# microsoft/Cream

Hardware: AMD Instinct MI355X
Metric: images/sec (whole node) AutoFormer-S supernet step @224^2 (higher is better)
Workload: dtype bf16; 1 GPU; AutoFormer-S supernet train step, random-path sampling (random.seed(epoch)), per-GPU batch 128, 224x224, AdamW, grad all-reduce RCCL; global_batch=128, parallelism=dp1, wgrad_partials=bf16 split-K partial tiles (within 1.9e-3 of fp32 partials), mixup=on-device, in the timed region

## Files before the change

cream_amd/_lib.py:

```python
import ctypes
import os

_HERE = os.path.dirname(os.path.abspath(__file__))
LIB_PATH = os.path.join(_HERE, "libcream_amd.so")

CREAM_OK = 0
_ERRORS = {
    -1: "CREAM_ERR_BAD_ARG (null pointer, negative size or unsupported stride)",
    -2: "CREAM_ERR_BAD_DTYPE (element type not supported by this entry point)",
    -3: "CREAM_ERR_LAUNCH (HIP kernel launch failed)",
    -4: "CREAM_ERR_TOO_LARGE (shape exceeds what the kernel family supports)",
    -5: "CREAM_ERR_CHANNEL_STRIDE (the channel stride of a (B, H, W, C) view is not 1)",
    -6: "CREAM_ERR_BAD_STRIDE (a stride is negative, not a multiple of 8, or tokens overlap)",
    -7: "CREAM_ERR_BAD_SHAPE (a channel count or a map size outside the covered range)",
}

F32, F16, BF16, F64 = 0, 1, 2, 3


class CreamLibraryError(RuntimeError):
    pass


_c = ctypes
# ... 50 lines not shown
    "cream_token_dwconv3_bwd": (_i, [_vp, _vp]),
    "cream_token_dwconv7_part_size": (_i, [_i]),
    "cream_token_dwconv7_blocks": (_i, [_vp]),
    "cream_token_dwconv7_fwd": (_i, [_vp, _vp]),
    "cream_token_dwconv7_bwd": (_i, [_vp, _vp]),
    "cream_cga_attn_check": (_i, [_vp]),
    "cream_cga_attn_fwd": (_i, [_vp, _vp]),
    "cream_evit_dwffn_check": (_i, [_vp]),
    "cream_evit_dwffn_fwd": (_i, [_vp, _vp]),
    "cream_evit_pw_residual_check": (_i, [_vp]),
    "cream_evit_pw_residual_fwd": (_i, [_vp, _vp]),
    "cream_relation_loss_check": (_i, [_vp]),
    "cream_relation_loss_blocks": (_i, [_vp]),
    "cream_relation_loss": (_i, [_vp, _vp]),
    "cream_hidden_relation_check": (_i, [_vp]),
    "cream_hidden_relation_padded": (_i, [_i]),
    "cream_hidden_relation_parts": (_i, [_i, _i]),
    "cream_hidden_relation_loss": (_i, [_vp, _vp]),
    "cream_attn_rpe2d_padded_len": (_i, [_i]),
    "cream_attn_rpe2d_dtab_parts": (_i, [_i, _i]),
    "cream_attn_rpe2d_bwd_mode": (_i, [_i]),
    "cream_attn_rpe2d_fwd": (_i, [_vp, _vp, _vp, _vp, _vp, _vp, _i64, _i64, _i64, _vp, _vp, _vp, _vp, _i,
                                  _i, _i, _i, _i, _i, _i, _f, _i, _vp]),
    "cream_attn_rpe2d_bwd": (_i, [_vp, _vp, _vp, _i64, _i64, _i64, _vp, _vp, _vp, _vp, _vp,
                                  _vp, _vp, _vp, _vp, _vp, _vp, _vp, _i64, _i64, _i64,
                                  _vp, _vp, _vp, _vp, _i, _i, _i, _i, _i, _i, _i, _f, _i, _vp]),
    "cream_attn_rpe2d_fwd_img": (_i, [_vp, _vp, _vp, _vp, _vp, _vp, _i64, _i64, _i64, _vp, _vp, _vp, _vp, _i, _vp,
                                      _i, _i, _i, _i, _i, _i, _f, _i, _vp]),
    "cream_attn_rpe2d_bwd_img": (_i, [_vp, _vp, _vp, _i64, _i64, _i64, _vp, _vp, _vp, _vp, _vp,
                                      _vp, _vp, _vp, _vp, _vp, _vp, _vp, _i64, _i64, _i64,
                                      _vp, _vp, _vp, _vp, _i, _vp, _i, _i, _i, _i, _i, _i, _f, _i, _vp]),
    "cream_attn_rpe2d_fwd_drop": (_i, [_vp, _vp, _vp, _vp, _vp, _vp, _i64, _i64, _i64, _vp, _vp, _vp, _vp, _i, _vp,
                                       _i, _i, _i, _i, _i, _i, _f, _f, _c.c_uint32, _i, _vp]),
    "cream_attn_rpe2d_bwd_drop": (_i, [_vp, _vp, _vp, _i64, _i64, _i64, _vp, _vp, _vp, _vp, _vp,
                                       _vp, _vp, _vp, _vp, _vp, _vp, _vp, _i64, _i64, _i64,
                                       _vp, _vp, _vp, _vp, _i, _vp, _i, _i, _i, _i, _i, _i, _f, _f, _c.c_uint32, _i, _vp]),
    "cream_attn_rpe2d_table_image_bytes": (_i64, []),
    "cream_attn_rpe2d_table_images": (_i, [_vp, _vp, _vp, _vp, _vp, _i, _i, _vp]),
    "cream_attn_rpe2d_fwd_mode": (_i, [_i]),
    "cream_ln_fwd": (_i, [_vp, _vp, _vp, _vp, _vp, _vp, _i, _i, _f, _vp]),
    "cream_ln_partials": (_i, []),
    "cream_ln_bwd": (_i, [_vp, _vp, _vp, _vp, _vp, _vp, _vp, _vp, _vp, _vp, _i, _i, _i, _vp]),
    "cream_gelu_fwd": (_i, [_vp, _vp, _i64, _vp]),
    "cream_gelu_bwd": (_i, [_vp, _vp, _vp, _i64, _vp]),
    "cream_residual_add": (_i, [_vp, _vp, _vp, _vp, _i64, _i64, _vp]),
    "cream_scale_cast": (_i, [_vp, _vp, _vp, _i64, _i64, _vp]),
    "cream_colsum_slabs": (_i, [_i]),
    "cream_colsum": (_i, [_vp, _vp, _i, _i, _vp]),
    "cream_add_ln_fwd": (_i, [_vp, _vp, _vp, _vp, _vp, _vp, _vp, _i, _vp, _vp, _i, _i, _f, _vp]),
    "cream_block_wgrad_bf16": (_i, [_i]),
    "cream_colsum128_slabs": (_i, [_i]),
    "cream_colsum128": (_i, [_vp, _vp, _i, _i, _vp]),
    "cream_gelu_bwd_colsum": (_i, [_vp, _vp, _vp, _vp, _i, _i, _vp]),
    "cream_scale_cast_colsum": (_i, [_vp, _vp, _vp, _vp, _i, _i, _i, _vp]),
    "cream_grad_finalize": (_i, [_vp, _i, _vp]),
    "cream_ln_fwd_masked": (_i, [_vp, _vp, _vp, _vp, _vp, _vp, _vp, _i, _i, _i, _f, _vp]),
    "cream_add_ln_fwd_masked": (_i, [_vp, _vp, _vp, _vp, _vp, _vp, _vp, _i, _vp, _vp, _vp, _i, _i, _i, _f, _vp]),
    "cream_ln_bwd_masked": (_i, [_vp, _vp, _vp, _vp, _vp, _vp, _vp, _vp, _vp, _i, _vp, _vp, _i, _i, _i, _vp]),
    "cream_mask_pack_check": (_i, [_vp, _i]),
    "cream_mask_pack": (_i, [_vp, _i, _vp]),
    "cream_mask_grad_ws_floats": (_i64, [_i, _i]),
    "cream_mask_grad_check": (_i, [_vp, _i]),
    "cream_mask_grad_finalize": (_i, [_vp, _i, _vp]),
    "cream_grad_finalize_compact_check": (_i, [_vp, _i]),
    "cream_grad_finalize_compact": (_i, [_vp, _i, _vp]),
    "cream_pad_cols": (_i, [_vp, _vp, _i, _i, _i, _i, _vp]),
    "cream_unpad_cols": (_i, [_vp, _i, _vp, _i, _i, _i, _vp]),
    "cream_gemm_rows_per_colsum_slab": (_i, []),
    "cream_gemm_nt256": (_i, [_i]),
    "cream_gemm_nt8": (_i, [_i]),
    "cream_linear_fwd": (_i, [_vp, _vp, _vp, _vp, _i, _i, _i, _i64, _vp]),
    "cream_linear_fwd_seg": (_i, [_vp, _vp, _vp, _vp, _i, _i, _i, _i64, _i, _i64, _vp]),
    "cream_linear_gelu_fwd": (_i, [_vp, _vp, _vp, _vp, _vp, _i, _i, _i, _i64, _vp]),
    "cream_linear_gelu_fwd_pad": (_i, [_vp, _vp, _vp, _vp, _vp, _i, _i, _i, _i, _i64, _vp]),
    "cream_linear_dgrad": (_i, [_vp, _vp, _vp, _i, _i, _i, _i64, _vp]),
    "cream_linear_dgrad_seg": (_i, [_vp, _vp, _vp, _i, _i, _i, _i64, _i, _i64, _vp]),
    "cream_linear_dgrad_mul": (_i, [_vp, _vp, _vp, _vp, _vp, _i, _i, _i, _i64, _vp]),
    "cream_linear_wgrad_splits": (_i, [_i, _i, _i]),
    "cream_linear_wgrad_splits_bf16": (_i, [_i, _i, _i]),
    "cream_gemm_tn8": (_i, [_i]),
    "cream_gemm_nthalf": (_i, [_i]),
    "cream_gemm_nt224": (_i, [_i]),
    "cream_gemm_nt224_launches": (_i64, []),
    "cream_linear_nt224": (_i, [_vp, _vp, _vp, _vp, _i, _i, _i, _i64, _i, _i64, _i, _i64, _vp]),
    "cream_gemm_ntopt": (_i, [_i]),
    "cream_gemm_stagger": (_i, [_i]),
    "cream_block_layout_epoch": (_i, []),
    "cream_cu_reserve": (_i, [_i]),
    "cream_mixup_cutmix": (_i, [_vp, _vp, _vp, _i, _i, _i, _i, _i, _f, _i, _i, _i, _i, _i, _f, _vp]),
    "cream_image_batch_plan": (_i64, [_vp, _i, _i, _i]),
    "cream_image_batch_transform": (_i, [_vp, _vp, _i64, _vp, _vp, _i, _i, _i, _vp, _vp, _vp, _i64, _vp]),
    "cream_cu_count": (_i, []),
    "cream_linear_wgrad_parts": (_i, [_vp, _vp, _vp, _vp, _i, _i, _i, _i, _vp]),
    "cream_linear_wgrad_parts_bf16": (_i, [_vp, _vp, _vp, _vp, _i, _i, _i, _i, _vp]),
    "cream_param_job_tiles": (_i, [_i, _i]),
    "cream_adamw_step": (_i, [_vp, _vp, _i, _i, _i, _c.c_double, _c.c_double, _c.c_double, _c.c_double, _i64, _vp]),
    "cream_grad_clip_coef": (_i, [_vp, _vp, _i, _i, _c.c_double, _vp, _vp, _vp]),
    "cream_adamw_step_clipped": (_i, [_vp, _vp, _i, _i, _i, _c.c_double, _c.c_double, _c.c_double, _c.c_double, _i64, _vp, _vp]),
    "cream_grad_scale": (_i, [_vp, _vp, _i, _i, _vp, _vp]),
    "cream_adamw_step_groups": (_i, [_vp, _vp, _i, _i, _i, _vp, _vp, _i, _c.c_double, _c.c_double, _c.c_double, _i64, _vp, _vp]),
    "cream_soft_ce": (_i, [_vp, _vp, _vp, _vp, _i, _i, _i, _f, _vp]),
    "cream_sparse_ce": (_i, [_vp, _vp, _vp, _vp, _vp, _i, _i, _i, _i, _f, _vp]),
    "cream_softmax_topk_records": (_i, [_vp, _vp, _vp, _i, _i, _i, _i, _vp]),
    "cream_linear_f32_fwd": (_i, [_vp, _vp, _vp, _vp, _i, _i, _i, _i64, _i64, _i, _i, _vp]),
    "cream_bmm_f32": (_i, [_vp, _vp, _vp, _i, _i, _i, _vp, _vp, _vp, _i, _i, _vp]),
    "cream_linear_f32_dgrad": (_i, [_vp, _vp, _vp, _i, _i, _i, _i64, _i, _i, _vp]),
    "cream_linear_f32_wgrad": (_i, [_vp, _vp, _vp, _vp, _i, _i, _i, _i64, _i64, _i, _i, _vp]),
    "cream_ln_f32_fwd": (_i, [_vp, _vp, _vp, _vp, _vp, _vp, _i, _i, _f, _vp]),
    "cream_ln_f32_bwd": (_i, [_vp, _vp, _vp, _vp, _vp, _vp, _vp, _i, _i, _vp]),
    "cream_block_prof_enable": (_i, [_i]),
    "cream_block_prof_kinds": (_i, []),
    "cream_block_prof_name": (_c.c_char_p, [_i]),
    "cream_block_prof_collect": (_i, [_vp, _vp, _vp, _vp]),
    "cream_slices_copy": (_i, [_vp, _i, _vp, _i, _i, _vp]),
    "cream_block_fwd_workspace": (_i64, [_vp, _vp, _vp, _vp]),
    "cream_block_fwd": (_i, [_vp, _vp, _vp, _vp, _vp, _vp, _vp]),
    "cream_block_bwd_workspace": (_i64, [_vp, _vp, _vp, _vp]),
    "cream_block_bwd": (_i, [_vp, _vp, _vp, _vp, _vp, _vp, _vp, _vp, _i, _i64, _vp, _vp, _i, _vp, _vp]),
    "cream_image_augment_workspace": (_i64, [_i, _i, _i, _i]),
    "cream_image_augment_u8": (_i, [_vp, _vp, _i, _i, _i, _vp, _vp, _i, _vp, _i64, _vp]),
    "cream_image_batch_plan_aug": (_i64, [_vp, _i, _i, _i, _vp, _i]),
    "cream_image_batch_transform_aug": (_i, [_vp, _vp, _i64, _vp, _vp, _i, _i, _i, _vp, _vp, _vp, _vp, _i, _vp, _i64, _vp]),
}

MAX_GRAD_JOBS = 24
ADAMW_MAX_GROUPS = 64


class GradJob(ctypes.Structure):
    _fields_ = [("dst", _vp), ("src", _vp), ("ld", _i64), ("pstride", _i64),
                ("nparts", _c.c_int32), ("rows", _c.c_int32), ("cols", _c.c_int32),
                ("interleave", _c.c_int32), ("src_bf16", _c.c_int32), ("overwrite", _c.c_int32)]

MAX_MASK_JOBS = 16


class MaskPackJob(ctypes.Structure):
    _fields_ = ([(n, _vp) for n in ("w", "r", "c", "mir", "mir_t")] + [(n, _i64) for n in ("ld", "ld_mir", "ld_mir_t")] +
                [(n, _c.c_int32) for n in ("rows", "cols", "c_group", "reserved")])


class MaskGradJob(ctypes.Structure):
    _fields_ = ([(n, _vp) for n in ("dst", "src", "w", "r", "c", "dr_out", "dc_out", "ws")] +
                [(n, _i64) for n in ("ld", "pstride", "ld_w")] +
                [(n, _c.c_int32) for n in ("nparts", "rows", "cols", "c_group", "src_bf16", "overwrite", "dr_accumulate",
                                           "dc_accumulate")])


MAX_COMPACT_JOBS = 24


class GradCompactJob(ctypes.Structure):
    _fields_ = ([("dst", _vp), ("src", _vp)] + [(n, _i64) for n in ("ld_dst", "ld_src", "pstride")] +
                [(n, _c.c_int32) for n in ("nparts", "rows", "cols", "src_bf16", "overwrite", "reserved")])


class ImageDesc(ctypes.Structure):
    _fields_ = ([("offset", _i64)] +
                [(n, _c.c_int32) for n in ("height", "width", "row_stride", "box_top", "box_left", "box_h", "box_w", "resized_h",
                                           "resized_w", "win_top", "win_left", "flip", "row0", "nrows")] +
                [("tmp_off", _i64)] +
                [(n, _c.c_int32) for n in ("erase_top", "erase_left", "erase_h", "erase_w")] +
                [("erase_seed", _c.c_uint32), ("reserved", _c.c_int32)])


class AugOp(ctypes.Structure):
# ... 181 lines not shown
```

cream_amd/csrc/gemm_mfma.hip:

```cpp
#include <hip/hip_runtime.h>
#include <stdint.h>
#include <stdlib.h>
#include <atomic>

#include "cream_amd.h"
#include "gemm_mfma.hpp"
#include "gemm_nt8.hpp"
#include "gemm_nt224.hpp"
#include "gemm_tn8.hpp"
#include "launch_ev.hpp"
#include "cu_budget.hpp"
#include "env_switch.hpp"

namespace {
std::atomic<int> g_cu_reserve{0};
std::atomic<int> g_layout_epoch{0};
int physical_cus()
{
    static int cus = 0;
    if (!cus) {
        int dev = 0;
        hipDeviceProp_t prop;
        if (hipGetDevice(&dev) == hipSuccess && hipGetDeviceProperties(&prop, dev) == hipSuccess) cus = prop.multiProcessorCount;
        if (cus <= 0) cus = 256;
    }
    return cus;
}
}
namespace cream {
int cu_count()
{
    int c = (physical_cus() - g_cu_reserve.load(std::memory_order_relaxed)) / 8 * 8;
    return c < 8 ? 8 : c;
}
}

namespace {
using namespace cream;
using namespace cream::gemm;

int num_cus() { return cream::cu_count(); }

EnvSwitch g_nt256{"CREAM_GEMM_NT256", 2};
int nt256_mode() { return g_nt256.get(); }

EnvSwitch g_ntopt{"CREAM_GEMM_NTOPT", 3, [](int m) { return m & 15; }};
int ntopt_mode() { return g_ntopt.get(); }
EnvSwitch g_stagger{"CREAM_GEMM_STAGGER", 0};
int stagger_mode() { return g_stagger.get(); }

template <int EPI>
int launch_nt256(const NtParams& p, hipStream_t st)
{
    constexpr int BM = 256, BN = 256;
    auto kern = (ntopt_mode() & 4) ? gemm_nt_kernel<BM, BN, 2, 4, 2, EPI, 1, 1> : gemm_nt_kernel<BM, BN, 2, 4, 2, EPI, 1>;
    constexpr int lds = nt_lds_bytes(BM, BN, 2);
    if (!cream::raise_dynamic_lds(kern, lds)) return CREAM_ERR_LAUNCH;
    const int tiles = ((p.M + BM - 1) / BM) * ((p.N + BN - 1) / BN), slots = num_cus() / 8 * 8;
    CREAM_LAUNCH(kern, dim3(tiles < slots ? tiles : slots), dim3(512), lds, st, p);
    return hipGetLastError() == hipSuccess ? CREAM_OK : CREAM_ERR_LAUNCH;
}

EnvSwitch g_nt8{"CREAM_GEMM_NT8", 4};
int nt8_mode() { return g_nt8.get(); }

bool nt8_fits(const NtParams& p)
{
    const int64_t amax = (int64_t)p.M * p.lda, bmax = (int64_t)2 * p.nseg_stride + (int64_t)p.nseg * p.ldb + p.ldb;
    const int64_t bplain = (int64_t)p.N * p.ldb;
    return amax < ((int64_t)1 << 31) && bmax < ((int64_t)1 << 31) && bplain < ((int64_t)1 << 31) && p.lda < (1 << 24) && p.ldb < (1 << 24);
}

template <int EPI>
int launch_nt8(const NtParams& p, hipStream_t st)
{
    auto kern = gemm_nt8_kernel<EPI>;
    if (!cream::raise_dynamic_lds(kern, NT8_LDS_BYTES)) return CREAM_ERR_LAUNCH;
    const int slots = num_cus() / 8 * 8;
    const int tiles = ((p.M + 255) / 256) * ((p.N + 255) / 256);
    CREAM_LAUNCH(kern, dim3(tiles < slots ? tiles : slots), dim3(512), NT8_LDS_BYTES, st, p);
    return hipGetLastError() == hipSuccess ? CREAM_OK : CREAM_ERR_LAUNCH;
}

EnvSwitch g_nthalf{"CREAM_GEMM_NTHALF", 1, norm_bool};
int nthalf_mode() { return g_nthalf.get(); }

template <int EPI, int BN, int WM, int WN>
int launch_nt_half(const NtParams& p, hipStream_t st)
{
    constexpr int BM = 256;
    auto kern = (ntopt_mode() & 4) ? gemm_nt_kernel<BM, BN, WM, WN, 2, EPI, 1, 1> : gemm_nt_kernel<BM, BN, WM, WN, 2, EPI, 1>;
    constexpr int lds = nt_lds_bytes(BM, BN, 2);
    if (!cream::raise_dynamic_lds(kern, lds)) return CREAM_ERR_LAUNCH;
    const int tiles = ((p.M + BM - 1) / BM) * ((p.N + BN - 1) / BN), slots = num_cus() / 8 * 8;
    CREAM_LAUNCH(kern, dim3(tiles < slots ? tiles : slots), dim3(WM * WN * 64), lds, st, p);
    return hipGetLastError() == hipSuccess ? CREAM_OK : CREAM_ERR_LAUNCH;
}

EnvSwitch g_nt224{"CREAM_GEMM_NT224", 1, norm_bool};
int nt224_mode() { return g_nt224.get(); }
std::atomic<int64_t> g_nt224_launches{0};

template <int EPI>
int launch_nt224(const NtParams& p, hipStream_t st)
{
    auto kern = gemm_nt224_kernel<EPI>;
    if (!cream::raise_dynamic_lds(kern, NT224_LDS_BYTES)) return CREAM_ERR_LAUNCH;
    const int tiles = ((p.M + NT224_BM - 1) / NT224_BM) * ((p.N + NT224_BN - 1) / NT224_BN), slots = num_cus() / 8 * 8;
    CREAM_LAUNCH(kern, dim3(tiles < slots ? tiles : slots), dim3(512), NT224_LDS_BYTES, st, p);
    g_nt224_launches.fetch_add(1, std::memory_order_relaxed);
    return hipGetLastError() == hipSuccess ? CREAM_OK : CREAM_ERR_LAUNCH;
}

template <int EPI>
int launch_nt(const NtParams& p, hipStream_t st)
{
    if constexpr (EPI == EPI_STORE || EPI == EPI_BIAS) {
        if (nt224_mode() > 0 && p.M >= 1024) {
            if (p.N == 448) return launch_nt224<EPI>(p, st);
            if (EPI == EPI_BIAS && p.N == 1344 && p.nseg == 448) return launch_nt224<EPI>(p, st);
        }
        if (nthalf_mode() > 0 && p.M >= 1024) {
            if (p.N == 384 || p.N == 320) return launch_nt_half<EPI, 192, 4, 2>(p, st);
        }
    }
    {
        const int m8 = nt8_mode();
        const bool light = EPI == EPI_STORE || EPI == EPI_BIAS;
        const int npad = (p.N + 255) / 256 * 256;
        if ((m8 == 1 || (m8 == 2 && (light || p.K >= 1024)) || (m8 == 3 && light && (npad - p.N) * 8 <= npad) ||
             (m8 == 4 && EPI == EPI_BIAS && (npad - p.N) * 8 <= npad) ||
             (m8 == 4 && p.K >= 640 && p.N >= 640)) && nt8_fits(p))
            return launch_nt8<EPI>(p, st);
    }
    {
        const int m256 = nt256_mode();
        if ((m256 == 1 && p.N >= 960) || (m256 == 2 && p.K >= 1152) || (m256 == 3 && p.K >= 960)) return launch_nt256<EPI>(p, st);
    }
    const int mode_ = ntopt_mode();
    const bool bwd_epi = EPI == EPI_MUL_COLSUM || EPI == EPI_STORE;
    const int opt = (bwd_epi && !(mode_ & 8)) ? 0 : mode_;
    if (p.N >= 640) {
        constexpr int BM = 128, BN = 128, OCC = 2;
        const int tiles = ((p.M + BM - 1) / BM) * ((p.N + BN - 1) / BN), slots = OCC * num_cus() / 8 * 8;
        NtParams q = p;
        q.stagger = tiles > slots / 2 ? stagger_mode() : 0;
        if (EPI == EPI_BIAS_GELU && (opt & 3) == 3) {
            auto kern = gemm_nt_kernel<BM, BN, 2, 2, 2, EPI, OCC, 3>;
            constexpr int lds = nt_lds_bytes(BM, BN, 2) + GELU_TAB_BYTES;
            if (!cream::raise_dynamic_lds(kern, lds)) return CREAM_ERR_LAUNCH;
            CREAM_LAUNCH(kern, dim3(tiles < slots ? tiles : slots), dim3(256), lds, st, q);
        } else if (opt & 1) {
            CREAM_LAUNCH((gemm_nt_kernel<BM, BN, 2, 2, 2, EPI, OCC, 1>), dim3(tiles < slots ? tiles : slots), dim3(256), 0, st, q);
        } else {
            CREAM_LAUNCH((gemm_nt_kernel<BM, BN, 2, 2, 2, EPI, OCC>), dim3(tiles < slots ? tiles : slots), dim3(256), 0, st, q);
        }
    } else {
        constexpr int BM = 128, BN = 64, OCC = 3;
        const int tiles = ((p.M + BM - 1) / BM) * ((p.N + BN - 1) / BN), slots = OCC * num_cus() / 8 * 8;
        if (opt & 1) {
            CREAM_LAUNCH((gemm_nt_kernel<BM, BN, 2, 2, 2, EPI, OCC, 1>), dim3(tiles < slots ? tiles : slots), dim3(256), 0, st, p);
        } else {
            CREAM_LAUNCH((gemm_nt_kernel<BM, BN, 2, 2, 2, EPI, OCC>), dim3(tiles < slots ? tiles : slots), dim3(256), 0, st, p);
        }
    }
    return hipGetLastError() == hipSuccess ? CREAM_OK : CREAM_ERR_LAUNCH;
}

bool aligned16(const void* p) { return ((uintptr_t)p & 15) == 0; }

int check_nt(const void* out, const void* a, const void* b, int M, int N, int K, int64_t ldb, int kmin_ld)
{
    if (M < 0 || N <= 0 || K <= 0 || ldb < kmin_ld) return CREAM_ERR_BAD_ARG;
    if (N % 8 || K % 8 || ldb % 8) return CREAM_ERR_BAD_ARG;
    if (M == 0) return 1;
    if (!out || !a || !b || !aligned16(out) || !aligned16(a) || !aligned16(b)) return CREAM_ERR_BAD_ARG;
    return CREAM_OK;
}

NtParams plain(void* out, const void* a, const void* b, int M, int N, int K, int64_t ldb)
{
    NtParams p{};
    p.A = (const uint16_t*)a; p.lda = K;
    p.B = (const uint16_t*)b; p.ldb = ldb;
    p.nseg = N; p.kseg = K; p.nseg_stride = 0; p.kseg_stride = 0;
    p.M = M; p.N = N; p.K = K;
    p.out = (uint16_t*)out; p.ldo = N;
    return p;
}

}

extern "C" {

int cream_gemm_rows_per_colsum_slab(void) { return 128; }

int cream_gemm_nt256(int on) { return g_nt256.set(on); }
int cream_gemm_nthalf(int on) { return g_nthalf.set(on); }
int cream_gemm_nt224(int on) { return g_nt224.set(on); }
int64_t cream_gemm_nt224_launches(void) { return g_nt224_launches.load(std::memory_order_relaxed); }
int cream_gemm_ntopt(int mode) { return g_ntopt.set(mode); }
int cream_gemm_stagger(int n) { return g_stagger.set(n); }
int cream_gemm_nt8(int mode) { return g_nt8.set(mode); }

int cream_linear_fwd(void* out, const void* x, const void* w, const void* bias, int M, int N, int K, int64_t ldw,
                     void* stream)
{
    const int rc = check_nt(out, x, w, M, N, K, ldw, K);
    if (rc) return rc < 0 ? rc : CREAM_OK;
    NtParams p = plain(out, x, w, M, N, K, ldw);
    p.bias = (const uint16_t*)bias;
    return launch_nt<EPI_BIAS>(p, (hipStream_t)stream);
}

int cream_linear_fwd_seg(void* out, const void* x, const void* w, const void* bias, int M, int N, int K, int64_t ldw,
                         int nseg, int64_t nseg_stride, void* stream)
{
    const int rc = check_nt(out, x, w, M, N, K, ldw, K);
    if (rc) return rc < 0 ? rc : CREAM_OK;
    if (nseg <= 0 || nseg % 8 || (int64_t)3 * nseg < N || nseg_stride % 8) return CREAM_ERR_BAD_ARG;
    NtParams p = plain(out, x, w, M, N, K, ldw);
    p.bias = (const uint16_t*)bias;
    p.nseg = nseg; p.nseg_stride = nseg_stride;
    return launch_nt<EPI_BIAS>(p, (hipStream_t)stream);
}

int cream_linear_nt224(void* out, const void* x, const void* w, const void* bias, int M, int N, int K, int64_t ldw, int nseg,
                       int64_t nseg_stride, int kseg, int64_t kseg_stride, void* stream)
{
    const int rc = check_nt(out, x, w, M, N, K, ldw, kseg > 0 && kseg < K ? kseg : K);
    if (rc) return rc < 0 ? rc : CREAM_OK;
    NtParams p = plain(out, x, w, M, N, K, ldw);
    if (nseg > 0) {
        if (nseg % 8 || (int64_t)3 * nseg < N || nseg_stride % 8) return CREAM_ERR_BAD_ARG;
        p.nseg = nseg; p.nseg_stride = nseg_stride;
    }
    if (kseg > 0) {
        if (kseg % 64 || K % kseg || kseg_stride % 8) return CREAM_ERR_BAD_ARG;
        p.kseg = kseg; p.kseg_stride = kseg_stride;
    }
    p.bias = (const uint16_t*)bias;
    return bias ? launch_nt224<EPI_BIAS>(p, (hipStream_t)stream) : launch_nt224<EPI_STORE>(p, (hipStream_t)stream);
}

int cream_linear_gelu_fwd_pad(void* gp, void* g, const void* x, const void* w, const void* bias, int M, int N, int Nvalid,
                              int K, int64_t ldw, void* stream)
{
    const int rc = check_nt(gp ? gp : g, x, w, M, N, K, ldw, K);
    if (rc) return rc < 0 ? rc : CREAM_OK;
    if (!g || !bias || !aligned16(g) || Nvalid <= 0 || Nvalid > N) return CREAM_ERR_BAD_ARG;
    NtParams p = plain(gp, x, w, M, N, K, ldw);
    p.bias = (const uint16_t*)bias;
    p.out2 = (uint16_t*)g;
    p.nvalid = Nvalid;
    return launch_nt<EPI_BIAS_GELU>(p, (hipStream_t)stream);
}

int cream_linear_gelu_fwd(void* gp, void* g, const void* x, const void* w, const void* bias, int M, int N, int K,
                          int64_t ldw, void* stream)
{
    return cream_linear_gelu_fwd_pad(gp, g, x, w, bias, M, N, N, K, ldw, stream);
}

int cream_linear_dgrad(void* dx, const void* dy, const void* wt, int M, int N, int K, int64_t ldwt, void* stream)
{
    const int rc = check_nt(dx, dy, wt, M, K, N, ldwt, N);
    if (rc) return rc < 0 ? rc : CREAM_OK;
    const NtParams p = plain(dx, dy, wt, M, K, N, ldwt);
    return launch_nt<EPI_STORE>(p, (hipStream_t)stream);
}

int cream_linear_dgrad_seg(void* dx, const void* dy, const void* wt, int M, int N, int K, int64_t ldwt, int kseg,
                           int64_t kseg_stride, void* stream)
{
    const int rc = check_nt(dx, dy, wt, M, K, N, ldwt, kseg);
    if (rc) return rc < 0 ? rc : CREAM_OK;
    if (kseg <= 0 || kseg % 64 || N % kseg || kseg_stride % 8) return CREAM_ERR_BAD_ARG;
    NtParams p = plain(dx, dy, wt, M, K, N, ldwt);
    p.kseg = kseg; p.kseg_stride = kseg_stride;
    return launch_nt<EPI_STORE>(p, (hipStream_t)stream);
}

int cream_linear_dgrad_mul(void* dh, float* colsum_parts, const void* dy, const void* wt, const void* factor, int M, int N,
                             int K, int64_t ldwt, void* stream)
{
    const int rc = check_nt(dh, dy, wt, M, K, N, ldwt, N);
    if (rc) return rc < 0 ? rc : CREAM_OK;
    if (!colsum_parts || !factor || !aligned16(factor)) return CREAM_ERR_BAD_ARG;
    NtParams p = plain(dh, dy, wt, M, K, N, ldwt);
    p.aux = (const uint16_t*)factor; p.ldaux = K;
    p.colsum = colsum_parts;
    return launch_nt<EPI_MUL_COLSUM>(p, (hipStream_t)stream);
}

}

namespace {
EnvSwitch g_tn8{"CREAM_GEMM_TN8", 2};
int tn8_mode() { return g_tn8.get(); }
int tn8_tiles(int N, int K) { return ((N + 255) / 256) * ((K + 255) / 256); }
int tn8_splits(int M, int N, int K)
{
    const int T = tn8_tiles(N, K), steps = (M + 63) / 64;
    static const int share = getenv("CREAM_WGRAD_CUS") ? atoi(getenv("CREAM_WGRAD_CUS")) : 0;
    int slots = num_cus() / 2 / 8 * 8;
    if (share >= 8) slots = (share < num_cus() ? share : num_cus()) / 8 * 8;
    int s = slots / T;
    if (s > steps) s = steps;
    return s < 1 ? 1 : s;
}
bool tn8_wanted(int M, int N, int K)
{
    const int mode = tn8_mode();
    if (mode <= 0 || M <= 0 || N % 8 || K % 8) return false;
    const int T = tn8_tiles(N, K);
    if ((int64_t)64 * (N > K ? N : K) * 2 + 4096 >= ((int64_t)1 << 31)) return false;
    return mode >= 2 ? T <= num_cus() : (T >= 6 && T <= num_cus());
}
}

extern "C" {

int cream_gemm_tn8(int mode)
{
    const int prev = g_tn8.set(mode);
// ... 81 lines not shown
```

include/cream_amd.h:

```cpp
#ifndef CREAM_AMD_H_
#define CREAM_AMD_H_

#include <stdint.h>

#ifdef __cplusplus
extern "C" {
#endif

#define CREAM_OK               0
#define CREAM_ERR_BAD_ARG     -1
#define CREAM_ERR_BAD_DTYPE   -2
#define CREAM_ERR_LAUNCH      -3
#define CREAM_ERR_TOO_LARGE   -4
#define CREAM_ERR_CHANNEL_STRIDE -5
#define CREAM_ERR_BAD_STRIDE  -6
#define CREAM_ERR_BAD_SHAPE   -7

#define CREAM_F32   0
#define CREAM_F16   1
#define CREAM_BF16  2
#define CREAM_F64   3

const char* cream_version(void);

// ... 332 lines not shown
    void *dq, *dk, *dv;
    int64_t dsb, dsn;
} cream_relation_desc;

int cream_relation_loss_check(const cream_relation_desc* d);

int cream_relation_loss_blocks(const cream_relation_desc* d);

int cream_relation_loss(const cream_relation_desc* d, void* stream);

typedef struct cream_hidden_relation_desc {
    const void *s, *t;
    int32_t s_dtype, t_dtype, B, L, Cs, Ct, want_grad;
    float coef;
    void *sn, *tn;
    float *s_rinv, *t_rinv, *g, *part;
    void* ds;
} cream_hidden_relation_desc;

int cream_hidden_relation_check(const cream_hidden_relation_desc* d);
int cream_hidden_relation_padded(int C);
int cream_hidden_relation_parts(int B, int L);
int cream_hidden_relation_loss(const cream_hidden_relation_desc* d, void* stream);

typedef struct cream_irpe_attn2_desc {
    cream_irpe_attn_desc base;
    int32_t head_dim;
    int32_t row_width;
    const uint8_t* key_pad;
    int64_t key_pad_sb;
    int64_t osb, osn, dosb, dosn;
} cream_irpe_attn2_desc;

int cream_irpe_attn2_check(const cream_irpe_attn2_desc* d, int backward);

int cream_irpe_attn2_fwd(const cream_irpe_attn2_desc* d, void* stream);

int cream_irpe_attn2_bwd(const cream_irpe_attn2_desc* d, void* stream);

int cream_irpe_table_grad2(float* out, const void* x, int64_t xsb, int64_t xsn, int64_t xsh, int xa, const void* y,
                           int64_t ysb, int64_t ysn, int64_t ysh, int yc, int B, int H, int L, float mul, void* stream);


int cream_ln_fwd(void* y, float* mean, float* rstd, const float* x, const float* gamma,
                 const float* beta, int M, int E, float eps, void* stream);

int cream_add_ln_fwd(float* xsum, void* y, float* mean, float* rstd, const float* x, const void* res,
                     const float* sample_scale, int rows_per_sample, const float* gamma,
                     const float* beta, int M, int E, float eps, void* stream);

int cream_ln_partials(void);

int cream_ln_bwd(float* dx, void* dx_scaled, float* partial, const void* dy, const float* x,
                 const float* mean, const float* rstd, const float* gamma, const float* dres,
                 const float* sample_scale, int rows_per_sample, int M, int E, void* stream);

int cream_gelu_fwd(void* g, const void* h, int64_t n, void* stream);
int cream_gelu_bwd(void* dh, const void* dg, const void* h, int64_t n, void* stream);

int cream_residual_add(float* out, const float* x, const void* y, const float* sample_scale,
                       int64_t n, int64_t per_sample, void* stream);

int cream_scale_cast(void* out, const float* x, const float* sample_scale, int64_t n,
                     int64_t per_sample, void* stream);

int cream_colsum_slabs(int M);
int cream_colsum(float* partial, const void* a, int M, int C, void* stream);

int cream_colsum128_slabs(int M);
int cream_colsum128(float* partial, const void* a, int M, int C, void* stream);
int cream_gelu_bwd_colsum(void* dh, float* partial, const void* dg, const void* h, int M, int C,
                          void* stream);
int cream_scale_cast_colsum(void* out, float* partial, const float* x, const float* sample_scale,
                            int rows_per_sample, int M, int C, void* stream);

int cream_gemm_rows_per_colsum_slab(void);

int cream_gemm_nt256(int on);
int cream_gemm_nthalf(int on);
int cream_gemm_nt224(int on);
int64_t cream_gemm_nt224_launches(void);
int cream_linear_nt224(void* out, const void* x, const void* w, const void* bias, int M, int N, int K, int64_t ldw, int nseg,
                       int64_t nseg_stride, int kseg, int64_t kseg_stride, void* stream);
int cream_gemm_nt8(int mode);
int cream_gemm_ntopt(int mode);
int cream_gemm_stagger(int n);
int cream_linear_fwd(void* out, const void* x, const void* w, const void* bias, int M, int N, int K,
                     int64_t ldw, void* stream);
int cream_linear_fwd_seg(void* out, const void* x, const void* w, const void* bias, int M, int N, int K,
                         int64_t ldw, int nseg, int64_t nseg_stride, void* stream);
int cream_linear_gelu_fwd(void* gp, void* g, const void* x, const void* w, const void* bias, int M, int N,
                          int K, int64_t ldw, void* stream);
int cream_linear_gelu_fwd_pad(void* gp, void* g, const void* x, const void* w, const void* bias, int M, int N, int Nvalid,
                              int K, int64_t ldw, void* stream);
int cream_linear_dgrad(void* dx, const void* dy, const void* wt, int M, int N, int K, int64_t ldwt,
                       void* stream);
int cream_linear_dgrad_seg(void* dx, const void* dy, const void* wt, int M, int N, int K, int64_t ldwt,
                           int kseg, int64_t kseg_stride, void* stream);
int cream_linear_dgrad_mul(void* dh, float* colsum_parts, const void* dy, const void* wt, const void* factor,
                             int M, int N, int K, int64_t ldwt, void* stream);
int cream_linear_wgrad_splits(int M, int N, int K);
int cream_linear_wgrad_parts(float* parts, float* bias_parts, const void* dy, const void* x, int M, int N,
                             int K, int S, void* stream);
int cream_linear_wgrad_parts_bf16(void* parts_bf16, float* bias_parts, const void* dy, const void* x, int M, int N,
                                  int K, int S, void* stream);
int cream_linear_wgrad_splits_bf16(int M, int N, int K);
int cream_gemm_tn8(int mode);

typedef struct cream_param_job {
    float* p;
    const float* g;
    float *m, *v;
    void *mir, *mir_t;
    int64_t ld, ld_mir, ld_mir_t, seg_stride, seg_stride_t;
    int32_t rows, cols, deinterleave;
    float weight_decay;
} cream_param_job;
int cream_param_job_tiles(int rows, int cols);
int cream_adamw_step(const cream_param_job* jobs_dev, const int32_t* first_tile_dev, int njobs, int total_tiles,
                     int update, double lr, double beta1, double beta2, double eps, int64_t step, void* stream);

int cream_grad_clip_coef(const cream_param_job* jobs_dev, const int32_t* first_tile_dev, int njobs, int total_tiles,
                         double max_norm, double* partials_dev, float* out_dev, void* stream);
int cream_adamw_step_clipped(const cream_param_job* jobs_dev, const int32_t* first_tile_dev, int njobs, int total_tiles,
                             int update, double lr, double beta1, double beta2, double eps, int64_t step,
                             const float* coef_dev, void* stream);
int cream_grad_scale(const cream_param_job* jobs_dev, const int32_t* first_tile_dev, int njobs, int total_tiles,
                     const float* coef_dev, void* stream);

#define CREAM_ADAMW_MAX_GROUPS 64
int cream_adamw_step_groups(const cream_param_job* jobs_dev, const int32_t* first_tile_dev, int njobs, int total_tiles,
                            int update, const int32_t* group_of_job_dev, const double* lr_of_group, int ngroups,
                            double beta1, double beta2, double eps, int64_t step, const float* coef_dev, void* stream);

typedef struct cream_grad_job {
    float* dst;
    const void* src;
    int64_t ld;
    int64_t pstride;
    int32_t nparts, rows, cols;
    int32_t interleave;
    int32_t src_bf16;
    int32_t overwrite;
} cream_grad_job;
#define CREAM_MAX_GRAD_JOBS 24
int cream_grad_finalize(const cream_grad_job* jobs, int njobs, void* stream);

int cream_ln_fwd_masked(void* y, float* mean, float* rstd, const float* x, const float* gamma, const float* beta,
                        const float* z, int n_keep, int M, int E, float eps, void* stream);
int cream_add_ln_fwd_masked(float* xsum, void* y, float* mean, float* rstd, const float* x, const void* res,
                            const float* sample_scale, int rows_per_sample, const float* gamma, const float* beta,
                            const float* z, int n_keep, int M, int E, float eps, void* stream);
int cream_ln_bwd_masked(float* dx, void* dx_scaled, float* partial, const void* dy, const float* x, const float* mean,
                        const float* rstd, const float* gamma, const float* z, int n_keep, const float* dres,
                        const float* sample_scale, int rows_per_sample, int M, int E, void* stream);

typedef struct cream_mask_pack_job {
    const float* w;
    const float* r;
    const float* c;
    void *mir, *mir_t;
    int64_t ld, ld_mir, ld_mir_t;
    int32_t rows, cols, c_group, reserved;
} cream_mask_pack_job;
#define CREAM_MAX_MASK_JOBS 16
int cream_mask_pack_check(const cream_mask_pack_job* jobs, int njobs);
// ... 170 lines not shown
```

Measured before the change: 14840 images/sec.

## Add persistent full-row-panel NT GEMM kernel for N=384/320 store GEMMs

Adds a persistent MFMA GEMM kernel that gives each workgroup a 256-row panel covering the full output width (384 or 320). It uses direct global-to-LDS DMA loads, double buffering, and prefetches the next panel while the current epilogue is stored through LDS staging. It becomes the default dispatch for EPI_STORE GEMMs with M>=1024 and N of 384 or 320, replacing the nthalf path. The intent is to load each A row once per panel, avoiding two half-width passes, and to overlap the epilogue with the next panel's loads. The cost is a large LDS footprint at one workgroup per CU and fewer concurrent workgroups.

New measurement: 15080 images/sec (median of 6 runs). +1.6%, better.

```diff
diff --git a/cream_amd/_lib.py b/cream_amd/_lib.py
--- a/cream_amd/_lib.py
+++ b/cream_amd/_lib.py
@@ -156,6 +156,9 @@
     "cream_gemm_nthalf": (_i, [_i]),
     "cream_gemm_nt224": (_i, [_i]),
     "cream_gemm_nt224_launches": (_i64, []),
+    "cream_gemm_ntrow": (_i, [_i]),
+    "cream_gemm_ntrow_launches": (_i64, []),
+    "cream_linear_ntrow": (_i, [_vp, _i64, _vp, _i64, _vp, _i, _i, _i, _i64, _i, _i64, _vp]),
     "cream_linear_nt224": (_i, [_vp, _vp, _vp, _vp, _i, _i, _i, _i64, _i, _i64, _i, _i64, _vp]),
     "cream_gemm_ntopt": (_i, [_i]),
     "cream_gemm_stagger": (_i, [_i]),
diff --git a/cream_amd/csrc/gemm_mfma.hip b/cream_amd/csrc/gemm_mfma.hip
--- a/cream_amd/csrc/gemm_mfma.hip
+++ b/cream_amd/csrc/gemm_mfma.hip
@@ -7,6 +7,7 @@
 #include "gemm_mfma.hpp"
 #include "gemm_nt8.hpp"
 #include "gemm_nt224.hpp"
+#include "gemm_ntrow.hpp"
 #include "gemm_tn8.hpp"
 #include "launch_ev.hpp"
 #include "cu_budget.hpp"
@@ -112,9 +113,36 @@
     return hipGetLastError() == hipSuccess ? CREAM_OK : CREAM_ERR_LAUNCH;
 }
 
+EnvSwitch g_ntrow{"CREAM_GEMM_NTROW", 1, norm_bool};
+int ntrow_mode() { return g_ntrow.get(); }
+std::atomic<int64_t> g_ntrow_launches{0};
+
+bool ntrow_fits(const NtParams& p)
+{
+    const int64_t amax = (int64_t)NTROW_BM * p.lda, bmax = (int64_t)2 * p.nseg_stride + (int64_t)p.nseg * p.ldb + p.ldb;
+    return p.lda > 0 && p.ldb > 0 && p.nseg_stride >= 0 && amax < ((int64_t)1 << 30) && bmax < ((int64_t)1 << 30) &&
+           (int64_t)p.N * p.ldb < ((int64_t)1 << 30);
+}
+
+template <int BN>
+int launch_ntrow(const NtParams& p, hipStream_t st)
+{
+    auto kern = gemm_ntrow_kernel<BN>;
+    constexpr int lds = ntrow_lds_bytes(BN);
+    if (!cream::raise_dynamic_lds(kern, lds)) return CREAM_ERR_LAUNCH;
+    const int panels = (p.M + NTROW_BM - 1) / NTROW_BM, slots = num_cus();
+    CREAM_LAUNCH(kern, dim3(panels < slots ? panels : slots), dim3(512), lds, st, p);
+    g_ntrow_launches.fetch_add(1, std::memory_order_relaxed);
+    return hipGetLastError() == hipSuccess ? CREAM_OK : CREAM_ERR_LAUNCH;
+}
+
 template <int EPI>
 int launch_nt(const NtParams& p, hipStream_t st)
 {
+    if constexpr (EPI == EPI_STORE) {
+        if (ntrow_mode() > 0 && p.M >= 1024 && (p.N == 384 || p.N == 320) && ntrow_fits(p))
+            return p.N == 384 ? launch_ntrow<384>(p, st) : launch_ntrow<320>(p, st);
+    }
     if constexpr (EPI == EPI_STORE || EPI == EPI_BIAS) {
         if (nt224_mode() > 0 && p.M >= 1024) {
             if (p.N == 448) return launch_nt224<EPI>(p, st);
@@ -199,6 +227,8 @@
 int cream_gemm_nthalf(int on) { return g_nthalf.set(on); }
 int cream_gemm_nt224(int on) { return g_nt224.set(on); }
 int64_t cream_gemm_nt224_launches(void) { return g_nt224_launches.load(std::memory_order_relaxed); }
+int cream_gemm_ntrow(int on) { return g_ntrow.set(on); }
+int64_t cream_gemm_ntrow_launches(void) { return g_ntrow_launches.load(std::memory_order_relaxed); }
 int cream_gemm_ntopt(int mode) { return g_ntopt.set(mode); }
 int cream_gemm_stagger(int n) { return g_stagger.set(n); }
 int cream_gemm_nt8(int mode) { return g_nt8.set(mode); }
@@ -241,6 +271,22 @@
     }
     p.bias = (const uint16_t*)bias;
     return bias ? launch_nt224<EPI_BIAS>(p, (hipStream_t)stream) : launch_nt224<EPI_STORE>(p, (hipStream_t)stream);
+}
+
+int cream_linear_ntrow(void* out, int64_t ldo, const void* x, int64_t ldx, const void* w, int M, int N, int K, int64_t ldw, int kseg,
+                       int64_t kseg_stride, void* stream)
+{
+    const int rc = check_nt(out, x, w, M, N, K, ldw, kseg > 0 && kseg < K ? kseg : K);
+    if (rc) return rc < 0 ? rc : CREAM_OK;
+    if ((N != 384 && N != 320) || ldo < N || ldo % 8 || ldx < K || ldx % 8) return CREAM_ERR_BAD_ARG;
+    NtParams p = plain(out, x, w, M, N, K, ldw);
+    p.lda = ldx; p.ldo = ldo;
+    if (kseg > 0) {
+        if (kseg % 64 || K % kseg || kseg_stride % 8) return CREAM_ERR_BAD_ARG;
+        p.kseg = kseg; p.kseg_stride = kseg_stride;
+    }
+    if (!ntrow_fits(p)) return CREAM_ERR_BAD_ARG;
+    return N == 384 ? launch_ntrow<384>(p, (hipStream_t)stream) : launch_ntrow<320>(p, (hipStream_t)stream);
 }
 
 int cream_linear_gelu_fwd_pad(void* gp, void* g, const void* x, const void* w, const void* bias, int M, int N, int Nvalid,
diff --git a/cream_amd/csrc/gemm_ntrow.hpp b/cream_amd/csrc/gemm_ntrow.hpp
--- /dev/null
+++ b/cream_amd/csrc/gemm_ntrow.hpp
@@ -0,0 +1,200 @@
+#pragma once
+#include "gemm_mfma.hpp"
+#include "gemm_nt8.hpp"
+
+namespace cream {
+namespace gemm {
+
+constexpr int NTROW_BM = 256;
+__host__ __device__ constexpr int ntrow_lds_bytes(int BN) { return nt_lds_bytes(NTROW_BM, BN, 2); }
+
+__device__ __forceinline__ void ntrow_dma(const void* base, uint32_t off, uint32_t lds_dst) {
+    uint32_t keep;
+    asm volatile("s_mov_b32 %0, m0\n\ts_mov_b32 m0, %2\n\ts_nop 0\n\tglobal_load_lds_dwordx4 %1, %3\n\ts_mov_b32 m0, %0"
+                 : "=&s"(keep) : "v"(off), "s"(lds_dst), "s"(base) : "memory");
+}
+
+template <int BN>
+__global__ __launch_bounds__(512, 1) void gemm_ntrow_kernel(const NtParams p)
+{
+    constexpr int BM = NTROW_BM, BK = 64, NW = 8;
+    constexpr int WTM = 64, WTN = BN / 2, TM = WTM / 32, TN = WTN / 32;
+    constexpr uint32_t STAGE_B = (BM + BN) * BK * 2;
+    constexpr int NPA = BM / 8 / NW, NPB = BN / 8 / NW;
+    constexpr int NCG = (TN + 1) / 2;
+    constexpr int NS = TM * (4 * (TN / 2) + 2 * (TN % 2));
+    static_assert(BN % 64 == 0 && (BN / 8) % NW == 0 && WTN % 32 == 0, "tile");
+    static_assert(NW * 4096 <= STAGE_B && NS <= 63, "epilogue staging inside stage 1; vmcnt immediate");
+    char* const smem = LdsBlock<ntrow_lds_bytes(BN)>::get();
+    const uint32_t lds0 = __builtin_amdgcn_readfirstlane((uint32_t)reinterpret_cast<uintptr_t>(smem));
+
+    const int tid = threadIdx.x, lane = tid & 63, g = lane >> 5, c32 = lane & 31;
+    const int wave = __builtin_amdgcn_readfirstlane(tid >> 6);
+    const int wm = wave >> 1, wn = wave & 1;
+    const int npanels = (p.M + BM - 1) / BM;
+    const int K = p.K, nfull = K / BK, rem = K % BK, nk = nfull + (rem ? 1 : 0);
+
+    const int prow = wave * 8 + (lane >> 3);
+    const int cch = ((lane & 7) ^ ((prow >> 1) & 7)) * 8;
+    uint32_t offA[NPA], offB[NPB];
+#pragma unroll
+    for (int j = 0; j < NPB; ++j) {
+        const int n = prow + 64 * j;
+        const int seg = (n >= p.nseg) + (n >= 2 * p.nseg);
+        offB[j] = (uint32_t)(seg * (int)p.nseg_stride + (n - seg * p.nseg) * (int)p.ldb + cch) * 2u;
+    }
+    auto here = [](uint32_t v) -> uint32_t { asm volatile("" : "+v"(v)); return v; };
+    auto lane_now = []() -> int {
+        uint32_t l;
+        asm volatile("v_mbcnt_lo_u32_b32 %0, -1, 0\n\tv_mbcnt_hi_u32_b32 %0, -1, %0" : "=v"(l));
+        return (int)l;
+    };
+    auto set_panel = [&](int m0) {
+        const int ln = lane_now(), pr = wave * 8 + (ln >> 3), ch = ((ln & 7) ^ ((pr >> 1) & 7)) * 8;
+#pragma unroll
+        for (int i = 0; i < NPA; ++i) offA[i] = (uint32_t)(min(pr + 64 * i, p.M - 1 - m0) * (int)p.lda + ch) * 2u;
+    };
+    int64_t kb = 0;
+    int kin = 0;
+    auto issue = [&](int m0, int k0, int buf, auto tail) {
+        const char* baseA = reinterpret_cast<const char*>(p.A + (int64_t)m0 * p.lda + k0);
+        const char* baseB = reinterpret_cast<const char*>(p.B + kb);
+        const uint32_t dst = lds0 + (uint32_t)buf * STAGE_B + (uint32_t)wave * 1024u;
+        const bool valid = k0 + cch < K;
+#pragma unroll
+        for (int i = 0; i < NPA; ++i) {
+            if constexpr (decltype(tail)::value)
+                nt8_dma(valid ? baseA + here(offA[i]) : reinterpret_cast<const char*>(g_nt8_zero), dst + (uint32_t)i * (NW * 1024u));
+            else ntrow_dma(baseA, offA[i], dst + (uint32_t)i * (NW * 1024u));
+        }
+#pragma unroll
+        for (int j = 0; j < NPB; ++j) {
+            if constexpr (decltype(tail)::value)
+                nt8_dma(valid ? baseB + here(offB[j]) : reinterpret_cast<const char*>(g_nt8_zero), dst + (uint32_t)(NPA + j) * (NW * 1024u));
+            else ntrow_dma(baseB, offB[j], dst + (uint32_t)(NPA + j) * (NW * 1024u));
+        }
+        kb += BK;
+        kin += BK;
+        if (kin >= p.kseg) { kin = 0; kb += p.kseg_stride - p.kseg; }
+    };
+    using No = std::integral_constant<bool, false>;
+    using Yes = std::integral_constant<bool, true>;
+    auto issue_step = [&](int m0, int s, int buf) { if (s < nfull) issue(m0, s * BK, buf, No{}); else issue(m0, s * BK, buf, Yes{}); };
+
+    const int sw = (c32 >> 1) & 7;
+    auto frag = [&](const char* tile, int row, int chunk) -> bf16x8 {
+        return *reinterpret_cast<const bf16x8*>(tile + row * (BK * 2) + ((chunk ^ sw) << 4));
+    };
+    f32x16 acc[TN][TM];
+    auto step = [&](int buf) {
+        const char* At = smem + (uint32_t)buf * STAGE_B;
+        const char* Bt = At + BM * BK * 2;
+        constexpr int NU = (BK / 16) * TN, AHEAD = 2;
+        bf16x8 fa[2][TM], fb[NU];
+        auto ra = [&](int ks) {
+#pragma unroll
+            for (int i = 0; i < TM; ++i) fa[ks & 1][i] = frag(At, wm * WTM + i * 32 + c32, ks * 2 + g);
+        };
+        auto rb = [&](int u) { fb[u] = frag(Bt, wn * WTN + (u % TN) * 32 + c32, (u / TN) * 2 + g); };
+        ra(0);
+#pragma unroll
+        for (int u = 0; u < AHEAD; ++u) rb(u);
+#pragma unroll
+        for (int u = 0; u < NU; ++u) {
+            if (u + AHEAD < NU) rb(u + AHEAD);
+            if (u % TN == TN - 3 && u / TN + 1 < BK / 16) ra(u / TN + 1);
+#pragma unroll
+            for (int tm = 0; tm < TM; ++tm)
+                acc[u % TN][tm] = __builtin_amdgcn_mfma_f32_32x32x16_bf16(fb[u], fa[(u / TN) & 1][tm], acc[u % TN][tm], 0, 0, 0);
+        }
+        __builtin_amdgcn_sched_group_barrier(0x100, TM + AHEAD, 0);
+#pragma unroll
+        for (int u = 0; u < NU; ++u) {
+            const int nrd = (u + AHEAD < NU ? 1 : 0) + ((u % TN == TN - 3 && u / TN + 1 < BK / 16) ? TM : 0);
+            __builtin_amdgcn_sched_group_barrier(0x008, 1, 0);
+            if (nrd == 1) __builtin_amdgcn_sched_group_barrier(0x100, 1, 0);
+            else if (nrd == TM) __builtin_amdgcn_sched_group_barrier(0x100, TM, 0);
+            else if (nrd == TM + 1) __builtin_amdgcn_sched_group_barrier(0x100, TM + 1, 0);
+            __builtin_amdgcn_sched_group_barrier(0x008, TM - 1, 0);
+        }
+    };
+
+    char* const stg = smem + STAGE_B + wave * 4096;
+
+    int panel = blockIdx.x, m0 = panel * BM;
+    set_panel(m0);
+    issue_step(m0, 0, 0);
+    bool epi_pending = false;
+
+    for (;;) {
+#pragma unroll
+        for (int a = 0; a < TN; ++a)
+#pragma unroll
+            for (int b = 0; b < TM; ++b) acc[a][b] = f32x16{0, 0, 0, 0, 0, 0, 0, 0, 0, 0, 0, 0, 0, 0, 0, 0};
+
+        for (int s = 0; s < nk; ++s) {
+            if (s == 0 && epi_pending) wait_vmcnt<NS>(); else wait_vmcnt<0>();
+            __builtin_amdgcn_s_barrier();
+            asm volatile("" ::: "memory");
+            if (s + 1 < nk) issue_step(m0, s + 1, (s + 1) & 1);
+            step(s & 1);
+            asm volatile("s_waitcnt lgkmcnt(0)" ::: "memory");
+        }
+
+        const int cur_m0 = m0;
+        const int next = panel + (int)gridDim.x;
+        const bool has_next = next < npanels;
+        nt_lds_barrier();
+        if (has_next) {
+            panel = next; m0 = next * BM;
+            set_panel(m0);
+            kb = 0; kin = 0;
+            issue_step(m0, 0, 0);
+        }
+
+        const bool full = cur_m0 + BM <= p.M;
+        const int el = lane_now(), eg = el >> 5, ec32 = el & 31;
+#pragma unroll
+        for (int tm = 0; tm < TM; ++tm) {
+#pragma unroll
+            for (int cg = 0; cg < NCG; ++cg) {
+                const int nb = (2 * cg + 2 <= TN) ? 2 : 1;
+                const int rowb = nb * 64;
+#pragma unroll
+                for (int b = 0; b < 2; ++b) {
+                    if (b >= nb) continue;
+                    const f32x16& av = acc[2 * cg + b][tm];
+                    uint32_t pk[8];
+#pragma unroll
+                    for (int r4 = 0; r4 < 4; ++r4)
+#pragma unroll
+                        for (int h = 0; h < 2; ++h) pk[2 * r4 + h] = f2bf_pair(av[4 * r4 + 2 * h], av[4 * r4 + 2 * h + 1]);
+#pragma unroll
+                    for (int j = 0; j < 2; ++j) {
+                        auto r0 = __builtin_amdgcn_permlane32_swap(pk[4 * j], pk[4 * j + 2], false, false);
+                        auto r1 = __builtin_amdgcn_permlane32_swap(pk[4 * j + 1], pk[4 * j + 3], false, false);
+                        const int chunk = b * 4 + 2 * j + eg;
+                        const int pos = nb == 2 ? (chunk ^ (ec32 & 7)) : (chunk ^ ((ec32 >> 1) & 3));
+                        *reinterpret_cast<u32x4v*>(stg + ec32 * rowb + (pos << 4)) = u32x4v{r0[0], r1[0], r0[1], r1[1]};
+                    }
+                }
+                const int cpr = nb * 4, rps = 64 / cpr;
+                const int rrow = el / cpr, rlc = el % cpr;
+                const int ncol = wn * WTN + cg * 64 + rlc * 8;
+#pragma unroll
+                for (int i = 0; i < 4; ++i) {
+                    if (i * rps >= 32) continue;
+                    const int rr = rrow + rps * i, m = cur_m0 + wm * WTM + tm * 32 + rr;
+                    const int pos = nb == 2 ? (rlc ^ (rr & 7)) : (rlc ^ ((rr >> 1) & 3));
+                    const u32x4v v = *reinterpret_cast<const u32x4v*>(stg + rr * rowb + (pos << 4));
+                    if (full || m < p.M) st_out16(p.out + (int64_t)m * p.ldo + ncol, v);
+                }
+            }
+        }
+        if (!has_next) break;
+        epi_pending = full;
+    }
+}
+
+}
+}
diff --git a/include/cream_amd.h b/include/cream_amd.h
--- a/include/cream_amd.h
+++ b/include/cream_amd.h
@@ -438,6 +438,10 @@
 int64_t cream_gemm_nt224_launches(void);
 int cream_linear_nt224(void* out, const void* x, const void* w, const void* bias, int M, int N, int K, int64_t ldw, int nseg,
                        int64_t nseg_stride, int kseg, int64_t kseg_stride, void* stream);
+int cream_gemm_ntrow(int on);
+int64_t cream_gemm_ntrow_launches(void);
+int cream_linear_ntrow(void* out, int64_t ldo, const void* x, int64_t ldx, const void* w, int M, int N, int K, int64_t ldw, int kseg,
+                       int64_t kseg_stride, void* stream);
 int cream_gemm_nt8(int mode);
 int cream_gemm_ntopt(int mode);
 int cream_gemm_stagger(int n);
```
